# Lillthorin/YoloLite-Official-Repo

Measured on AMD Instinct MI355X. Metric: images/sec, higher is better.
Workload: dtype f32

## Files before the change

include/yololite_hip.h:

```cpp
#ifndef YOLOLITE_HIP_H
#define YOLOLITE_HIP_H

#include <stdint.h>

#ifdef __cplusplus
extern "C" {
#endif

#define YL_ABI_VERSION 7
#define YL_MAX_LEVELS 8

typedef struct yl_ctx yl_ctx;
typedef int32_t yl_status;

enum {
  YL_OK = 0,
  YL_ERR_INVALID = -1,
  YL_ERR_HIP = -2,
  YL_ERR_NOMEM = -3,
  YL_ERR_STATE = -4,
  YL_ERR_UNSUPPORTED = -5,
  YL_ERR_CAPACITY = -6
};

// ... 88 lines not shown

yl_status yl_create(const yl_model_desc* desc, int32_t device_id, yl_ctx** out);
yl_status yl_clone(const yl_ctx* src, yl_ctx** out);
yl_status yl_streams_overlap(int32_t device_id, void* a, void* b, int32_t* overlap);
void yl_destroy(yl_ctx* ctx);
const char* yl_strerror(yl_status s);
const char* yl_last_error(const yl_ctx* ctx);
int32_t yl_abi_version(void);

yl_status yl_forward(yl_ctx* ctx, const float* x_dev, int32_t batch, float* const* level_out_dev,
                     void* stream);
yl_status yl_forward_timed(yl_ctx* ctx, const float* x_dev, int32_t batch, float* const* level_out_dev,
                           void* stream, float* layer_ms);
yl_status yl_last_timing(yl_ctx* ctx, float* infer_ms, float* post_ms);
int64_t yl_activation_bytes(const yl_ctx* ctx);
yl_status yl_read_slot(yl_ctx* ctx, int32_t slot, int32_t batch, float* dst_dev, void* stream);
yl_status yl_set_option(yl_ctx* ctx, const char* name, int32_t value);
yl_status yl_get_option(const yl_ctx* ctx, const char* name, int32_t* value);
int32_t yl_query_fused_block(int32_t c_in, int32_t c_mid, int32_t c_out, int32_t dw_k, int32_t dw_stride, int32_t out_h,
                             int32_t out_w);
int32_t yl_query_ir_form(int32_t c_in, int32_t c_mid, int32_t c_out, int32_t dw_k, int32_t dw_stride, int32_t out_h, int32_t out_w,
                         int32_t batch, int32_t in_h, int32_t in_w, int32_t up_h, int32_t up_w, int32_t act, int32_t dw_act,
                         int32_t act2, int32_t* shape);
int32_t yl_query_dw_prologue(int32_t c_in, int32_t c_out, int32_t dw_k, int32_t dw_stride, int32_t out_h, int32_t out_w);
int32_t yl_query_wino_form(int32_t c_in, int32_t c_out, int32_t out_h, int32_t out_w, int32_t batch, int32_t in_shift,
                           int32_t dev_select, int32_t* mt, int32_t* nt);

typedef struct {
  int64_t offset;
  int32_t h0, w0;
  int32_t nh, nw;
  int32_t top, left;
} yl_pre_image;
yl_status yl_preprocess(yl_ctx* ctx, const uint8_t* packed_u8_dev, const yl_pre_image* imgs_dev, int32_t batch,
                        float* x_dev, void* stream);

yl_status yl_decode(yl_ctx* ctx, const float* const* levels_dev, int32_t batch, int32_t center_mode,
                    int32_t wh_mode, float* box_dev, float* obj_dev, float* cls_dev, void* stream);

yl_status yl_forward_decoded(yl_ctx* ctx, const float* x_dev, int32_t batch, int32_t center_mode, int32_t wh_mode,
                             float* box_dev, float* obj_dev, float* cls_dev, void* stream);

yl_status yl_postprocess(yl_ctx* ctx, const float* const* levels_dev, int32_t batch,
                         const yl_post_cfg* cfg, float* dets_dev, int32_t* counts_dev,
                         int32_t* keep_idx_dev, void* stream);
yl_status yl_predict(yl_ctx* ctx, const float* x_dev, int32_t batch, const yl_post_cfg* cfg,
// ... 424 lines not shown
```

yololite-official-repo_amd/_lib.py:

```python
from __future__ import annotations

import ctypes as C
import os
import sys
import warnings


def _default_hw_queues():
    if "GPU_MAX_HW_QUEUES" in os.environ or os.environ.get("YOLOLITE_NO_ENV_DEFAULTS"):
        return
    os.environ["GPU_MAX_HW_QUEUES"] = "8"
    t = sys.modules.get("torch")
    try:
        late = t is not None and t.cuda.is_initialized()
    except Exception:
        late = False
    if late:
        warnings.warn("yololite_amd: the HIP runtime was initialised before this package was imported, so "
                      "GPU_MAX_HW_QUEUES=8 cannot be applied; export it in the environment (multi-stream overlap "
                      "of the executor degrades by ~25 % next to RCCL streams otherwise)", RuntimeWarning)


_default_hw_queues()

_HERE = os.path.dirname(os.path.abspath(__file__))
LIB_PATH = os.environ.get("YOLOLITE_HIP_LIB") or os.path.join(_HERE, "libyololite_hip.so")

YL_ABI_VERSION = 7
YL_MAX_LEVELS = 8
YL_OK = 0
ACT = {"none": 0, "relu": 1, "relu6": 2, "silu": 3, "gelu": 4, "relu_lab": 5}
OP_STEM, OP_CONV, OP_DW, OP_STEMBLOCK, OP_SE = 0, 1, 2, 3, 4
OP_POOL, OP_COPY, OP_LN, OP_GRN, OP_NHWC4 = 5, 6, 7, 8, 9
POST_MAIN, POST_FALLBACK, POST_EVAL = 0, 1, 2
CENTER = {"v8": 0, "simple": 1}
WH = {"softplus": 0, "v8": 1, "exp": 2}
NMS_TORCHVISION, NMS_GREEDY = 0, 1

DEV_DW_TILE_OFF, DEV_PWS_OFF, DEV_S2C_OFF, DEV_DWC_ALL, DEV_DWT_OFF = 1, 2, 4, 8, 16
DEV_DWT_NOSPLIT = 1 << 10
DEV_WINO_V1 = 1 << 11
DEV_DWL_OFF = 1 << 14
DEV_DWL_ALL = 1 << 15
DEV_DPW_OFF = 1 << 16
DEV_K3W_OFF = 1 << 17
DEV_POISON = 1 << 18
DEV_CHAIN_OFF = 1 << 19
DEV_HEAD_SKIP_OFF = 1 << 20
DEV_PWX_OFF = 1 << 21
DEV_WINO_SHAPE_SHIFT = 12

_fp = C.POINTER(C.c_float)
_ip = C.POINTER(C.c_int32)


class yl_layer(C.Structure):
    _fields_ = [(n, C.c_int32) for n in (
        "op", "in_slot", "out_slot", "res_slot", "up_slot", "head_level", "cin", "cout",
        "k", "stride", "pad_t", "pad_l", "act", "in_shift", "dw_k", "dw_stride", "dw_pad_t", "dw_pad_l", "dw_act")] + [
        ("w", _fp), ("b", _fp), ("dw_w", _fp), ("dw_b", _fp),
        ("c2", C.c_int32), ("act2", C.c_int32), ("c3", C.c_int32), ("act3", C.c_int32),
        ("w2", _fp), ("b2", _fp), ("w3", _fp), ("b3", _fp), ("scale_slot", C.c_int32), ("reserved0", C.c_int32),
        ("lab_scale", C.c_float), ("lab_bias", C.c_float), ("eps", C.c_float), ("out_ch_off", C.c_int32)]


class yl_model_desc(C.Structure):
    _fields_ = [("abi_version", C.c_int32), ("img_size", C.c_int32), ("in_channels", C.c_int32),
                ("num_classes", C.c_int32), ("num_masks", C.c_int32), ("proto_slot", C.c_int32),
                ("num_levels", C.c_int32),
                ("level_size", C.c_int32 * YL_MAX_LEVELS), ("level_anchors", C.c_int32 * YL_MAX_LEVELS),
                ("num_slots", C.c_int32), ("slot_h", _ip), ("slot_w", _ip), ("slot_c", _ip),
                ("num_layers", C.c_int32), ("layers", C.POINTER(yl_layer))]
# ... 189 lines not shown


_vp = C.c_void_p
_vpp = C.POINTER(C.c_void_p)
SYMBOLS = [
    ("yl_create", C.c_int32, [C.POINTER(yl_model_desc), C.c_int32, C.POINTER(_vp)]),
    ("yl_clone", C.c_int32, [_vp, C.POINTER(_vp)]),
    ("yl_streams_overlap", C.c_int32, [C.c_int32, _vp, _vp, C.POINTER(C.c_int32)]),
    ("yl_destroy", None, [_vp]),
    ("yl_strerror", C.c_char_p, [C.c_int32]),
    ("yl_last_error", C.c_char_p, [_vp]),
    ("yl_abi_version", C.c_int32, []),
    ("yl_forward", C.c_int32, [_vp, _vp, C.c_int32, _vpp, _vp]),
    ("yl_forward_timed", C.c_int32, [_vp, _vp, C.c_int32, _vpp, _vp, _fp]),
    ("yl_last_timing", C.c_int32, [_vp, _fp, _fp]),
    ("yl_activation_bytes", C.c_int64, [_vp]),
    ("yl_read_slot", C.c_int32, [_vp, C.c_int32, C.c_int32, _vp, _vp]),
    ("yl_set_option", C.c_int32, [_vp, C.c_char_p, C.c_int32]),
    ("yl_get_option", C.c_int32, [_vp, C.c_char_p, _ip]),
    ("yl_query_fused_block", C.c_int32, [C.c_int32] * 7),
    ("yl_query_dw_prologue", C.c_int32, [C.c_int32] * 6),
    ("yl_query_wino_form", C.c_int32, [C.c_int32] * 7 + [_ip, _ip]),
    ("yl_query_ir_form", C.c_int32, [C.c_int32] * 15 + [_ip]),
    ("yl_forward_decoded", C.c_int32, [_vp, _vp, C.c_int32, C.c_int32, C.c_int32, _vp, _vp, _vp, _vp]),
    ("yl_preprocess", C.c_int32, [_vp, _vp, _vp, C.c_int32, _vp, _vp]),
    ("yl_decode", C.c_int32, [_vp, _vpp, C.c_int32, C.c_int32, C.c_int32, _vp, _vp, _vp, _vp]),
    ("yl_postprocess", C.c_int32, [_vp, _vpp, C.c_int32, C.POINTER(yl_post_cfg), _vp, _vp, _vp, _vp]),
    ("yl_predict", C.c_int32, [_vp, _vp, C.c_int32, C.POINTER(yl_post_cfg), _vp, _vp, _vp, _vp]),
    ("yl_allgather_dets", C.c_int32, [_vp, _vp, _vp, C.c_int64, _vp, _vp]),
    ("yl_masks", C.c_int32, [_vp, _vpp, C.c_int32, _vp, _vp, C.c_int32, C.c_float, _vp, _vp]),
    ("yl_masks_image", C.c_int32, [_vp, _vpp, C.c_int32, _vp, _vp, _vp, C.c_int32, C.c_float, _vp, _vp, _vp, C.c_int32,
                                   C.c_int32, C.c_int32, _vp, _vp]),
    ("yl_nms", C.c_int32, [_vp, _vp, _vp, C.c_int32, C.c_float, C.c_int32, C.c_int32, _vp, _vp, _vp]),
    ("yl_eval_match", C.c_int32, [_vp, _vp, _vp, _vp, C.c_int32, C.c_int32, C.c_double, _vp, _vp, _vp, _vp]),
    ("yl_eval_sweep", C.c_int32, [_vp, _vp, _vp, C.c_int32, _vp, C.c_int32, _vp, _vp, _vp]),
    ("yl_eval_confusion", C.c_int32, [_vp, _vp, _vp, _vp, _vp, _vp, C.c_int32, C.c_int32, C.c_int32, C.c_float,
                                      _vp, _vp, _vp]),
    ("yl_eval_coco_match", C.c_int32, [_vp, _vp, _vp, _vp, _vp, _vp, C.c_int32, C.c_int32, C.c_int32, _vp, C.c_int32,
                                       _vp, C.c_int32, _vp, _vp, _vp]),
    ("yl_eval_coco_accumulate", C.c_int32, [_vp, _vp, _vp, _vp, C.c_int32, _vp, C.c_int32, C.c_int32, C.c_int32, _vp,
                                            C.c_int32, _vp, C.c_int32, _vp, _vp, _vp]),
    ("yl_loss_af", C.c_int32, [_vp, _vpp, C.c_int32, _vp, _vp, _vp, C.c_int32, C.POINTER(yl_loss_cfg), _vp, _vp, _vp, _vp]),
    ("yl_loss_af_train", C.c_int32, [_vp, _vpp, C.c_int32, _vp, _vp, _vp, C.c_int32, C.POINTER(yl_loss_cfg), _vp, _vp, _vp,
                                     _vp, _vp]),
    ("yl_loss_af_backward", C.c_int32, [_vp, _vpp, C.c_int32, _vp, _vp, _vp, C.c_int32, C.POINTER(yl_loss_cfg), _vp, _vp,
                                        _vp, _vpp, _vp]),
# ... 48 lines not shown
                                       _ip]),
    ("yl_stem_plan", C.c_int32, [C.POINTER(yl_stem_cfg), C.c_int32, C.c_int32, C.POINTER(yl_stem_plan_info)]),
    ("yl_stem_create", C.c_int32, [C.c_int32, C.POINTER(yl_stem_cfg), C.POINTER(_vp)]),
    ("yl_stem_destroy", None, [_vp]),
    ("yl_stem_held", C.c_int32, [_vp, C.POINTER(C.c_int64), C.POINTER(C.c_int64), _ip]),
    ("yl_stem_forward", C.c_int32, [_vp, C.POINTER(yl_stem_tensors), _vp, C.c_int32, C.c_int32, C.c_uint32, _vp, _vp, _ip]),
    ("yl_stem_backward", C.c_int32, [_vp, C.POINTER(yl_stem_tensors), C.POINTER(yl_stem_tensors), _vp, _vp, _vp, _ip]),
    ("yl_stem_conv", C.c_int32, [_vp, _vp, _vp] + [C.c_int32] * 8 + [_vp, _ip]),
    ("yl_amp_stage_set", C.c_int32, [_vp, C.c_uint32]),
    ("yl_amp_stem_set", C.c_int32, [_vp, C.c_uint32]),
    ("yl_amp_stage_get", C.c_int32, [_vp, C.POINTER(C.c_uint32), C.POINTER(C.c_uint32)]),
    ("yl_amp_stem_get", C.c_int32, [_vp, C.POINTER(C.c_uint32), C.POINTER(C.c_uint32)]),
    ("yl_amp_stem_conv", C.c_int32, [_vp, _vp, _vp] + [C.c_int32] * 8 + [C.c_uint32, _vp, _ip]),
    ("yl_variant_stage_set", C.c_int32, [_vp, C.c_int32, C.c_int32]),
    ("yl_variant_stage_get", C.c_int32, [_vp, _ip, _ip]),
    ("yl_variant_stage_depthwise", C.c_int32, [_vp, _vp, _vp, C.c_int32, C.c_int32, C.c_int32, C.c_int32, C.c_int32, C.c_int32,
                                               C.c_int32, _vp, _ip]),
    ("yl_augment", C.c_int32, [_vp, _vp, _vp, C.c_int32, C.c_int32, _vp, _vp]),
]
SYMBOLS_DIGITS = [
    ("yl_dneck_conv3x3", C.c_int32, [_vp, C.c_int32, C.c_uint32, _vp, _vp, _vp, C.c_int32, C.c_int32, _vp, _ip]),
]

_lib = None


class YoloLiteHipError(RuntimeError):
    pass


def load():
    global _lib
    if _lib is not None:
        return _lib
    if not os.path.exists(LIB_PATH):
        raise YoloLiteHipError(
            f"{LIB_PATH} not found: build it with `python yololite-official-repo_amd/csrc/build.py` "
            "(or __graft_entry__.build()). There is no CPU fallback.")
    import torch
    try:
        lib = C.CDLL(LIB_PATH, mode=C.RTLD_GLOBAL)
    except OSError as e:
        raise YoloLiteHipError(f"cannot load {LIB_PATH}: {e}") from e
    for name, res, args in SYMBOLS + SYMBOLS_DIGITS:
        fn = getattr(lib, name)
        fn.restype = res
        fn.argtypes = args
    if lib.yl_abi_version() != YL_ABI_VERSION:
        raise YoloLiteHipError("libyololite_hip.so ABI version mismatch")
    _lib = lib
    return lib


def check(status: int, ctx=None, what: str = ""):
    if status == YL_OK:
        return
    lib = load()
    msg = lib.yl_strerror(status).decode()
    detail = lib.yl_last_error(ctx).decode() if ctx else ""
    raise YoloLiteHipError(f"{what or 'yololite_hip'}: {msg} ({status}) {detail}".strip())
```

yololite-official-repo_amd/csrc/yl_api.hip:

```cpp
#include "yl_internal.h"
#include "yl_program.h"

#include <dlfcn.h>
#include <limits.h>
#include <math.h>
#include <stdio.h>
#include <stddef.h>
#include <string.h>

#include <algorithm>
#include <memory>
#include <chrono>
#include <string>
#include <vector>

namespace {

struct DevLayer : YlLayerInfo {
#define YL_X(name) float* name = nullptr;
  YL_LAYER_IMAGES(YL_X)
#undef YL_X
};

struct Slot {
// ... 1227 lines not shown
    unsigned v = 0;
    if (c->head_skip_cnt &&
        (hipSetDevice(c->m->device) != hipSuccess || hipDeviceSynchronize() != hipSuccess ||
         hipMemcpy(&v, c->head_skip_cnt, sizeof(v), hipMemcpyDeviceToHost) != hipSuccess))
      return YL_ERR_HIP;
    *value = (int32_t)(v & 0x7fffffffu);
    return YL_OK;
  }
  return YL_ERR_INVALID;
}

int32_t yl_query_fused_block(int32_t c_in, int32_t c_mid, int32_t c_out, int32_t dw_k, int32_t dw_stride, int32_t out_h,
                             int32_t out_w) {
  if (c_in < 1 || c_mid < 1 || c_out < 1 || out_h < 1 || out_w < 1) return 0;
  if (yl_ir_supported(c_in, c_mid, c_out, dw_k, dw_stride, out_h, out_w)) return 1;
  if (dw_stride == 1 && !(out_h & 3) && !(out_w & 3) && yl_uib_supported(c_in, c_mid, c_out, dw_k)) return 2;
  return 0;
}

int32_t yl_query_ir_form(int32_t c_in, int32_t c_mid, int32_t c_out, int32_t dw_k, int32_t dw_stride, int32_t out_h, int32_t out_w,
                         int32_t batch, int32_t in_h, int32_t in_w, int32_t up_h, int32_t up_w, int32_t act, int32_t dw_act,
                         int32_t act2, int32_t* shape) {
  if (c_in < 1 || c_mid < 1 || c_out < 1 || out_h < 1 || out_w < 1 || batch < 1 || in_h < 1 || in_w < 1 || up_h < 0 || up_w < 0) return 0;
  return yl_ir_form(c_in, c_mid, c_out, dw_k, dw_stride, out_h, out_w, batch, in_h, in_w, up_h, up_w, act, dw_act, act2, shape);
}

int32_t yl_query_dw_prologue(int32_t c_in, int32_t c_out, int32_t dw_k, int32_t dw_stride, int32_t out_h, int32_t out_w) {
  if (c_in < 1 || c_out < 1 || dw_k < 1 || dw_stride < 1 || out_h < 1 || out_w < 1) return 0;
  if (yl_dws_supported(c_in, c_out, dw_k, dw_stride, out_h, out_w)) return 2;
  if ((size_t)(dw_k * dw_k + 1) * c_in * sizeof(float) <= YL_DW_LDS_MAX) return 1;
  return 0;
}

int32_t yl_query_wino_form(int32_t c_in, int32_t c_out, int32_t out_h, int32_t out_w, int32_t batch, int32_t in_shift,
                           int32_t dev_select, int32_t* mt, int32_t* nt) {
  if (mt) *mt = 0;
  if (nt) *nt = 0;
  if (c_in < 16 || c_out < 16 || (c_in & 3) || (c_out & 3)) return 0;
  const unsigned dev = (unsigned)dev_select;
  const YlWinoForm f = yl_wino_form(c_in, c_out, out_h, out_w, batch, in_shift, sizeof(float), (dev & YL_DEV_WINO_V1) != 0, YL_DEV_WINO_SHAPE(dev));
  if (f.form == 2) {
    if (mt) *mt = f.mt;
    if (nt) *nt = f.nt;
  }
  return f.form;
}

// ... 304 lines not shown
```

yololite-official-repo_amd/csrc/yl_convc.hip:

```cpp
#include "yl_lp.h"
#if YL_BF16
#define yl_conv_dwc_kernel YL_LP_NAME(yl_conv_dwc_kernel)
#define yl_launch_conv_dwc YL_LP_NAME(yl_launch_conv_dwc)
#define yl_convc_init YL_LP_NAME(yl_convc_init)
#define yl_conv_pwt_kernel YL_LP_NAME(yl_conv_pwt_kernel)
#define yl_launch_conv_pwt YL_LP_NAME(yl_launch_conv_pwt)
#define yl_launch_conv_pwt_multi YL_LP_NAME(yl_launch_conv_pwt_multi)
#define yl_conv_dwt_kernel YL_LP_NAME(yl_conv_dwt_kernel)
#define yl_launch_conv_dwt YL_LP_NAME(yl_launch_conv_dwt)
#define yl_conv_dwk_kernel YL_LP_NAME(yl_conv_dwk_kernel)
#define yl_conv_dwl_kernel YL_LP_NAME(yl_conv_dwl_kernel)
#define yl_launch_conv_dwk YL_LP_NAME(yl_launch_conv_dwk)
#define yl_conv_dws_kernel YL_LP_NAME(yl_conv_dws_kernel)
#define yl_launch_conv_dws YL_LP_NAME(yl_launch_conv_dws)
#define yl_conv_wino_kernel YL_LP_NAME(yl_conv_wino_kernel)
#define yl_launch_conv_wino YL_LP_NAME(yl_launch_conv_wino)
#define yl_conv_kxk_kernel YL_LP_NAME(yl_conv_kxk_kernel)
#define yl_launch_conv_kxk YL_LP_NAME(yl_launch_conv_kxk)
#define yl_conv_pws_kernel YL_LP_NAME(yl_conv_pws_kernel)
#define yl_launch_conv_pws YL_LP_NAME(yl_launch_conv_pws)
#define yl_ir_kernel YL_LP_NAME(yl_ir_kernel)
#define yl_launch_conv_ir YL_LP_NAME(yl_launch_conv_ir)
#define yl_ir_supported YL_LP_NAME(yl_ir_supported)
#define yl_ir_form YL_LP_NAME(yl_ir_form)
// ... 1324 lines not shown
  const int gy = (p.NTtot + NT - 1) / NT;
  const bool eight = ((long)p.M / 128) * gy >= 2 * 2 * YL_NUM_CU;
  return pws_go(p, st, cand, eight);
}

constexpr __host__ __device__ int yl_ir_pitch(int dk, int ds, int mt, int cbn) { return ((((4 * mt * cbn - 1) * ds + dk) * 16 + 7) / 64) * 64 + 56; }
constexpr __host__ __device__ int yl_ir_slab(int dk, int ds, int mt, int rbn, int cbn) { return ((4 * rbn - 1) * ds + dk) * yl_ir_pitch(dk, ds, mt, cbn); }
struct YlIrLds {
  static constexpr size_t LIMIT = 150 * 1024;
  size_t wpl, dwl, b2l, bytes;
  constexpr __host__ __device__ YlIrLds(int dk, int ds, int mt, int rbn, int cbn, int nt, int KB)
      : wpl((size_t)2 * yl_ir_slab(dk, ds, mt, rbn, cbn)), dwl(wpl + (size_t)2 * nt * 256), b2l(dwl + (size_t)KB * (dk * dk + 1) * 16),
        bytes((b2l + (size_t)KB * 16) * 4) {}
};

template <bool CLAMP>
__device__ __forceinline__ f32x4 yl_ir_act(f32x4 v, int act, float lo, float hi) {
  if constexpr (CLAMP) return yl_clamp4(v, lo, hi);
  else return yl_actc(v, act, lo, hi);
}
constexpr int yl_ir_waves(int kbi, int nt, int dk, int ds, int mt, bool clamp) {
  return (dk == 3 && ds * mt <= 2 && kbi <= 3 && (nt <= 3 || (clamp && ds * mt == 1))) ? 3 : 2;
}
template <int KBI , int NT, int DK, int DS, int MT, int RBN , int CBN , bool CLAMP>
__global__ __launch_bounds__(RBN * CBN * 64, yl_ir_waves(KBI, NT, DK, DS, MT, CLAMP)) void yl_ir_kernel(YlConvP p) {
  constexpr int NWV = RBN * CBN, NTH = NWV * 64;
  constexpr int TH = 4 * RBN, TW = 4 * MT * CBN;
  constexpr int HH = (TH - 1) * DS + DK, HW = (TW - 1) * DS + DK, HN = HH * HW;
  constexpr int HMT = (HN + 15) / 16, HMW = (HMT + NWV - 1) / NWV;
  constexpr int PITCHF = yl_ir_pitch(DK, DS, MT, CBN), SLAB = yl_ir_slab(DK, DS, MT, RBN, CBN);
  extern __shared__ __attribute__((aligned(16))) float yl_clds[];
  const int tid = threadIdx.x, lane = tid & 63;
  const int wave = __builtin_amdgcn_readfirstlane(tid >> 6);
  const int kq = lane >> 4, pl = lane & 15;
  const int Cmid = p.Cin, KB = p.KB, NTtot = p.NTtot, C1 = p.C1, H = p.H, W = p.W, OH = p.OH, OW = p.OW, N = p.N;
  const YlIrLds L(DK, DS, MT, RBN, CBN, NT, KB);
  float* slab = yl_clds;
  f32x4* wpl = reinterpret_cast<f32x4*>(yl_clds + L.wpl);
  float* dwl = yl_clds + L.dwl;
  float* b2l = yl_clds + L.b2l;
  const f32x4* wg = reinterpret_cast<const f32x4*>(p.wp);
  const f32x4* w2g = reinterpret_cast<const f32x4*>(p.w2p);
  const yl_act_t* const xin = p.x;
  const yl_act_t* const up = p.up;
  {
    constexpr int T1 = DK * DK + 1;
    for (int i = tid; i < KB * T1 * 16; i += NTH) {
      const int kb = i / (T1 * 16), r = i - kb * (T1 * 16), t = r >> 4, ch = kb * 16 + (r & 15);
// ... 105 lines not shown
      for (int nt = 0; nt < NT; ++nt) {
        acc[mt][nt] = (f32x4){0.f, 0.f, 0.f, 0.f};
        const int n = nt * 16 + 4 * kq;
        if (pre_add && n < N) acc[mt][nt] = yl_ld4(p.res + px[mt].lin * N + n);
      }
    f32x4 we[KBI], wn[KBI];
#pragma unroll
    for (int kbi = 0; kbi < KBI; ++kbi) {
      if constexpr (CLAMP) wn[kbi] = __builtin_bit_cast(f32x4, __builtin_amdgcn_raw_buffer_load_b128(wrs, lane16, kbi * KB * 1024, 0));
      else wn[kbi] = w2g[((size_t)kbi * KB + 0) * 64 + lane];
    }
    f32x4 un[HMW];
    auto load_up = [&](int kb, int j) {
      if constexpr (CLAMP) {
        return bld4(urs, (kb + 1 < KB || kb * 16 + 4 * kq < Cmid) ? uo[j] : OOR, kb * 16 * ESZ);
      } else {
        return yl_ld4((h_in[j] && kb * 16 + 4 * kq < Cmid) ? up + uoff[j] + kb * 16 : p.zeros);
      }
    };
    if (up) {
#pragma unroll
      for (int j = 0; j < HMW; ++j) un[j] = load_up(0, j);
    }
    for (int kb = 0; kb < KB; ++kb, ++gs) {
      const int buf = (int)(gs & 1u);
#pragma unroll
      for (int kbi = 0; kbi < KBI; ++kbi) we[kbi] = wn[kbi];
      if (kb + 1 < KB) {
#pragma unroll
        for (int kbi = 0; kbi < KBI; ++kbi) {
          if constexpr (CLAMP) wn[kbi] = __builtin_bit_cast(f32x4, __builtin_amdgcn_raw_buffer_load_b128(wrs, lane16, (kbi * KB + kb + 1) * 1024, 0));
          else wn[kbi] = w2g[((size_t)kbi * KB + kb + 1) * 64 + lane];
        }
      }
      const f32x4 eb = yl_ld4(b2l + kb * 16 + 4 * kq);
      float* sb = slab + buf * SLAB;
#pragma unroll
      for (int j = 0; j < HMW; ++j) {
        f32x4 e[1][1] = {{{0.f, 0.f, 0.f, 0.f}}};
        if (up) e[0][0] = un[j];
#pragma unroll
        for (int kbi = 0; kbi < KBI; ++kbi) {
          const f32x4 wq1[1] = {we[kbi]};
          const f32x4 xq1[1] = {xh[j][kbi]};
          yl_mma_step<1, 1>(wq1, xq1, e);
        }
// ... 15 lines not shown
#pragma unroll
          for (int mt = 0; mt < MT; ++mt) {
            const f32x4 v = *reinterpret_cast<const f32x4*>(sb + rbase + dy * PITCHF + (dx + 4 * mt * DS) * 16);
            xq[mt].x = fmaf(v.x, w.x, xq[mt].x); xq[mt].y = fmaf(v.y, w.y, xq[mt].y);
            xq[mt].z = fmaf(v.z, w.z, xq[mt].z); xq[mt].w = fmaf(v.w, w.w, xq[mt].w);
          }
        }
      };
#pragma unroll 1
      for (int dy = 0; dy < DK; ++dy) tap_row(dy);
#pragma unroll
      for (int mt = 0; mt < MT; ++mt) xq[mt] = yl_ir_act<CLAMP>(xq[mt], dw_act, dlo, dhi);
      f32x4 wq[NT];
      const f32x4* wrow = wpl + (size_t)buf * NT * 64 + lane;
#pragma unroll
      for (int nt = 0; nt < NT; ++nt) wq[nt] = wrow[nt * 64];
      yl_mma_step<NT, MT>(wq, xq, acc);
    }
    if (!pre_add && (p.res || (!CLAMP && YL_SMOOTH(p.act)))) yl_epi_generic<NT, MT>(p, acc, px, 0, kq);
    else yl_epi_fast<NT, MT>(p, acc, px, 0, kq, lo, hi, true);
  }
}

template <int KBI, int NT, int DK, int DS, int MT, int RBN, int CBN, bool CLAMP>
static hipError_t ir_go(const YlConvP& p, hipStream_t st, bool second) {
  if (CLAMP && !second) return hipErrorNotSupported;
  const size_t lds = YlIrLds(DK, DS, MT, RBN, CBN, NT, p.KB).bytes;
  const long ntiles = (long)p.B * (p.OH / (4 * RBN)) * (p.OW / (4 * MT * CBN));
  int gx = yl_resident_blocks((const void*)yl_ir_kernel<KBI, NT, DK, DS, MT, RBN, CBN, CLAMP>, RBN * CBN * 64, lds, 8);
  if (gx > ntiles) gx = (int)ntiles;
  if (gx >= 8) gx &= ~7;
  hipLaunchKernelGGL((yl_ir_kernel<KBI, NT, DK, DS, MT, RBN, CBN, CLAMP>), dim3(gx), dim3(RBN * CBN * 64), lds, st, p);
  return hipGetLastError();
}

#define YL_IR_SHAPES(X)                                                                                              \
  X(1, 2, 3, 2, 1, 2, 2) X(2, 2, 3, 1, 2, 2, 2) X(2, 3, 5, 2, 1, 2, 2) X(3, 3, 5, 1, 2, 2, 2) X(3, 6, 3, 2, 1, 2, 2)    \
  X(3, 3, 3, 1, 1, 2, 2) X(2, 6, 3, 1, 2, 2, 2) X(3, 6, 3, 1, 1, 2, 2)
#define YL_IR_BUCKET_LO(B) ((B) == 2 ? 0 : (B) == 3 ? 2 : (B) == 4 ? 3 : 4)

bool yl_ir_supported(int c1, int cmid, int n, int dk, int ds, int oh, int ow) {
  const int kbi = (c1 + 15) / 16, nt = (n + 15) / 16;
#define YL_IR_CHECK(A, B, C, D, E, R, S)                                                                             \
  if (kbi == A && nt <= B && nt > YL_IR_BUCKET_LO(B) && dk == C && ds == D && (oh % (4 * R)) == 0 &&                    \
      (ow % (4 * E * S)) == 0 && YlIrLds(C, D, E, R, S, B, (cmid + 15) / 16).bytes <= YlIrLds::LIMIT) return true;
  YL_IR_SHAPES(YL_IR_CHECK)
#undef YL_IR_CHECK
  return false;
}

int yl_ir_form(int c1, int cmid, int n, int dk, int ds, int oh, int ow, int batch, int h, int w, int uh, int uw, int act,
               int dw_act, int act2, int* shape) {
  const int kbi = (c1 + 15) / 16, nt = (n + 15) / 16, KB = (cmid + 15) / 16;
  const size_t lim = ((size_t)1 << 31) - 4096, e = sizeof(yl_act_t);
  const bool second = !YL_SMOOTH(act) && !YL_SMOOTH(dw_act) && !YL_SMOOTH(act2) && batch > 0 && h > 0 && w > 0 && uh >= 0 && uw >= 0 &&
                      (size_t)batch * h * w * c1 * e < lim && (size_t)batch * uh * uw * cmid * e < lim &&
                      (size_t)kbi * KB * 1024 < lim && (size_t)KB * nt * 1024 < lim;
#define YL_IR_FORM(A, B, C, D, E, R, S)                                                                              \
  if (kbi == A && nt <= B && nt > YL_IR_BUCKET_LO(B) && dk == C && ds == D && (oh % (4 * R)) == 0 &&                    \
      (ow % (4 * E * S)) == 0 && YlIrLds(C, D, E, R, S, B, KB).bytes <= YlIrLds::LIMIT) {                                \
    const int sh[7] = {A, B, C, D, E, R, S};                                                                         \
    for (int i = 0; shape && i < 7; ++i) shape[i] = sh[i];                                                           \
    return second ? 2 : 1;                                                                                           \
  }
  YL_IR_SHAPES(YL_IR_FORM)
#undef YL_IR_FORM
  return 0;
}

hipError_t yl_launch_conv_ir(const YlConvP& p, hipStream_t st) {
  if (p.C1 <= 0 || p.k != 1 || p.dw_k == 0 || (p.N & 3)) return hipErrorNotSupported;
  const int kbi = (p.C1 + 15) / 16, nt = p.NTtot;
  const bool second = yl_ir_form(p.C1, p.Cin, p.N, p.dw_k, p.dw_stride, p.OH, p.OW, p.B, p.H, p.W, p.up ? p.UH : 0, p.up ? p.UW : 0,
                                 p.act, p.dw_act, p.act2, nullptr) == 2;
#define YL_IR_RUN(A, B, C, D, E, R, S)                                                                               \
  if (kbi == A && nt <= B && nt > YL_IR_BUCKET_LO(B) && p.dw_k == C && p.dw_stride == D && (p.OH % (4 * R)) == 0 &&     \
      (p.OW % (4 * E * S)) == 0 && YlIrLds(C, D, E, R, S, B, p.KB).bytes <= YlIrLds::LIMIT) {                               \
    const hipError_t e2 = ir_go<A, B, C, D, E, R, S, true>(p, st, second);                                           \
    return e2 != hipErrorNotSupported ? e2 : ir_go<A, B, C, D, E, R, S, false>(p, st, second);                        \
  }
  YL_IR_SHAPES(YL_IR_RUN)
#undef YL_IR_RUN
  return hipErrorNotSupported;
}

struct YlDwkLds {
  static constexpr size_t LIMIT = 96 * 1024;
  static constexpr __host__ __device__ int steps(int NT, int GW) { return GW == 1 ? 3 : (GW * NT <= 16 ? 2 : 1); }
  size_t dwl, bytes;
  constexpr __host__ __device__ YlDwkLds(int NT, int GW, int Cin)
      : dwl((size_t)2 * steps(NT, GW) * GW * NT * 256), bytes((dwl + yl_taps_floats(3, Cin)) * 4) {}
};

template <int NT, int GW, int NW>
__global__ __launch_bounds__(NW * 64, GW == 1 ? 3 : 2) void yl_conv_dwk_kernel(YlConvP p) {
  constexpr int S = YlDwkLds::steps(NT, GW);
  constexpr int PCS = S * GW * NT;
// ... 1073 lines not shown
  const int gx = yl_band_grid(yl_resident_blocks((const void*)wino2_kernel_of(MT, NT, 0), 512, lds, 8), (long)p.ntiles * G);
  hipLaunchKernelGGL(wino2_kernel_of(MT, NT, p.in_shift), dim3(gx), dim3(512), lds, st, p);
  return hipGetLastError();
}

hipError_t yl_launch_conv_wino(const YlConvP& p, hipStream_t st) {
  if (!p.wino || p.k != 3 || p.stride != 1 || p.dw_k > 0 || p.up || p.dec_boxes || p.C1 > 0 || p.w3p || p.scale) return hipErrorNotSupported;
  const YlWinoForm f = yl_wino_form(p.Cin, p.N, p.OH, p.OW, p.B,
                                    p.in_shift, sizeof(yl_act_t), (p.dev & YL_DEV_WINO_V1) != 0, YL_DEV_WINO_SHAPE(p.dev));
  if (f.form == 0) return hipErrorNotSupported;
  return f.form == 2 ? wino2_go(p, st, f.mt, f.nt) : wino_go(p, st);
}

namespace {

#define YL_DWC_SHAPES(NTW) \
  {{yl_conv_dwc_kernel<3, 1, NTW>, yl_conv_dwc_kernel<3, 2, NTW>}, {yl_conv_dwc_kernel<5, 1, NTW>, yl_conv_dwc_kernel<5, 2, NTW>}}
const YlMultiKernel dwc_kernels[5][2][2] = {YL_DWC_SHAPES(1), YL_DWC_SHAPES(2), YL_DWC_SHAPES(3), YL_DWC_SHAPES(4), YL_DWC_SHAPES(5)};

int kbmax_of(int ntw) { return ntw == 1 ? 18 : ntw == 2 ? 9 : ntw == 3 ? 6 : 4; }

}

hipError_t yl_convc_init() {
  hipError_t e = hipSuccess;
  const auto cap = [&e](const auto& kernels, size_t bytes) { if (e == hipSuccess) e = yl_set_lds_cap(kernels, bytes); };
#define YL_KXK_CAP(A, B, C) cap(yl_conv_kxk_kernel<A, B, C>, YlKxkLds::LIMIT);
  YL_KXK_SHAPES(YL_KXK_CAP)
#define YL_IR_CAP(A, B, C, D, E, R, S) cap(yl_ir_kernel<A, B, C, D, E, R, S, false>, YlIrLds::LIMIT); cap(yl_ir_kernel<A, B, C, D, E, R, S, true>, YlIrLds::LIMIT);
  YL_IR_SHAPES(YL_IR_CAP)
  cap(pws_kernels, YlPwsLds::LIMIT);
  cap(pws_dec_kernels, YlPwsLds::LIMIT);
  cap(dwt_kernels, YlDwtLds::LIMIT);
  cap(dwt_splitk_kernels, YlDwtLds::LIMIT);
  cap(wino_kernels, YlWinoLds::LIMIT);
#define YL_WINO2_CAP(A, B) cap(yl_conv_wino2_kernel<A, B, 1>, YlWino2Lds(A).bytes); cap(yl_conv_wino2_kernel<A, B, 0>, YlWino2Lds(A).bytes);
  YL_WINO2_SHAPES(YL_WINO2_CAP)
#define YL_DWK_CAP(A, B, C) cap(yl_conv_dwk_kernel<A, B, C>, YlDwkLds::LIMIT);
  YL_DWK_SHAPES(YL_DWK_CAP)
#define YL_DWL_CAP(A) cap(yl_conv_dwl_kernel<A>, YlDwlLds::LIMIT);
  YL_DWL_SHAPES(YL_DWL_CAP)
#define YL_DWS_CAP(A, G, K, S_) cap(yl_conv_dws_kernel<A, G, K, S_, 4>, YlDwsLds::LIMIT);
  YL_DWS_SHAPES(YL_DWS_CAP)
#if !YL_BF16
#define YL_DWX_CAP(A, B) cap(yl_conv_dwx_kernel<A, B>, YlDwtLds::LIMIT);
  YL_DWX_SHAPES(YL_DWX_CAP)
#define YL_PWX_CAP(A, B, C, D) cap(yl_conv_pwx_kernel<A, B, C, D>, YlPwxLds::LIMIT);
  YL_PWX_SHAPES(YL_PWX_CAP)
#undef YL_PWX_CAP
#endif
  cap(dwc_kernels, YlDwcLds::LIMIT);
  return e;
// ... 37 lines not shown
```

yololite-official-repo_amd/csrc/yl_internal.h:

```cpp
#pragma once
#include <hip/hip_runtime.h>
#include <stdint.h>
#include <map>
#include <mutex>
#include <type_traits>
#include <utility>
#include "../../include/yololite_hip.h"
#include "yl_lp.h"
#include "yl_shapes.h"

#define YL_LDS_KEYS_MAX 16384

struct YlLevels {
  const float* ptr[YL_MAX_LEVELS];
  int S[YL_MAX_LEVELS];
  int A[YL_MAX_LEVELS];
  int off[YL_MAX_LEVELS + 1];
  float stride[YL_MAX_LEVELS];
  int L, N, E, C;
  float hi;
};

struct YlDecodeP {
  int mode;
// ... 115 lines not shown
  int ldo;
  int out_f32;
};

#define YL_DEV_DW_TILE_OFF (1u << 0)
#define YL_DEV_PWS_OFF (1u << 1)
#define YL_DEV_S2C_OFF (1u << 2)
#define YL_DEV_DWC_ALL (1u << 3)
#define YL_DEV_DWT_OFF (1u << 4)
#define YL_DEV_DWK(d) (((d) >> 5) & 3u)
#define YL_DEV_KXK_NW(d) (((d) >> 7) & 3u)
#define YL_DEV_KXK_MT2 (1u << 9)
#define YL_DEV_DWT_NOSPLIT (1u << 10)
#define YL_DEV_WINO_V1 (1u << 11)
#define YL_DEV_WINO_SHAPE(d) (((d) >> 12) & 3u)
#define YL_DEV_DWL_OFF (1u << 14)
#define YL_DEV_DWL_ALL (1u << 15)
#define YL_DEV_DPW_OFF (1u << 16)
#define YL_DEV_K3W_OFF (1u << 17)
#define YL_DEV_POISON (1u << 18)
#define YL_DEV_CHAIN_OFF (1u << 19)
#define YL_DEV_HEAD_SKIP_OFF (1u << 20)
#define YL_DEV_PWX_OFF (1u << 21)
#define YL_DEV_MASK 0x3ffffffu
static_assert(YL_DEV_MASK <= 0x7fffffffu, "dev_select is stored in an int (and an int field of the graph key)");
static_assert(((YL_DEV_DW_TILE_OFF | YL_DEV_PWS_OFF | YL_DEV_S2C_OFF | YL_DEV_DWC_ALL | YL_DEV_DWT_OFF | (3u << 5) | (3u << 7) |
                YL_DEV_KXK_MT2 | YL_DEV_DWT_NOSPLIT | YL_DEV_WINO_V1 | (3u << 12) | YL_DEV_DWL_OFF | YL_DEV_DWL_ALL | YL_DEV_DPW_OFF |
                YL_DEV_K3W_OFF | YL_DEV_POISON | YL_DEV_CHAIN_OFF | YL_DEV_HEAD_SKIP_OFF | YL_DEV_PWX_OFF) & ~YL_DEV_MASK) == 0, "a YL_DEV_* bit lies outside the dev_select mask");

struct YlSeP {
  const float* x;
  float* partial;
  const float* w1;
  const float* b1;
  const float* w2;
  const float* b2;
  float* gate;
  int B, HW, C, RD, P, act;
};
hipError_t yl_launch_se(const YlSeP& p, bool pooled, hipStream_t st);
int yl_se_parts(int HW, int C);
int yl_dw_pool_wpi(int k, int stride, int cin, int n, int oh, int ow);

struct YlOpP {
  const float* x;
  float* out;
  const float* w;
  const float* b;
  float* partial;
  int B, H, W, C, OH, OW;
  int k, stride, pad_t, pad_l;
// ... 123 lines not shown
```

yololite-official-repo_amd/csrc/yl_shapes.h:

```cpp
#pragma once

#define YL_SMOOTH(a) ((a) >= YL_ACT_SILU)
#define YL_ACT_POSTPASS(a) ((a) >= YL_ACT_GELU)

#include <stddef.h>

#define YL_NUM_CU 256

bool yl_stemblock_supported(int c1, int c2, int c3);
bool yl_uib_supported(int c1, int cmid, int n, int dk);
bool yl_ir_supported(int c1, int cmid, int n, int dk, int ds, int oh, int ow);
int yl_ir_form(int c1, int cmid, int n, int dk, int ds, int oh, int ow, int batch, int h, int w, int uh, int uw, int act,
               int dw_act, int act2, int* shape);
bool yl_dws_supported(int cin, int n, int dk, int ds, int oh, int ow);

#define YL_WINO2_SHAPES(X) X(4, 3) X(4, 4) X(2, 3) X(2, 4) X(2, 7)

struct YlWinoForm {
  int form;
  int mt, nt;
};

inline YlWinoForm yl_wino_form(int cin, int n, int oh, int ow, int batch, int in_shift, size_t elem, bool v1, unsigned shape) {
  if (cin < 1 || n < 1 || oh < 1 || ow < 1 || batch < 1 || (n & 3) || in_shift < 0 || in_shift > 1 ||
      ((size_t)batch * (oh >> in_shift) * (ow >> in_shift) * cin + (size_t)(ow + 1) * cin) * elem >= ((size_t)1 << 31))
    return {0, 0, 0};
  const int KB = (cin + 15) / 16, NTtot = (n + 15) / 16;
  const bool small = (size_t)batch * (oh >> in_shift) * (ow >> in_shift) * cin * elem < ((size_t)1 << 31) &&
                     (size_t)((NTtot + 1) / 2) * KB * 32768 < ((size_t)1 << 31);
  if (!v1 && KB >= 2 && NTtot >= 3 && small) {
    const int TW = (ow + 1) >> 1, TH = (oh + 1) >> 1;
    const int MX = (TW + 3) >> 2, MY = (TH + 3) >> 2;
    const long MTOT = (long)batch * MX * MY;
    if ((long)TW * TH * 100 >= (long)MX * MY * 16 * 65) {
      const int pad3 = (NTtot + 2) / 3 * 3, pad4 = (NTtot + 3) / 4 * 4;
      int nt = pad3 <= pad4 ? 3 : 4;
// ... 10 lines not shown
```

Before: 51750.

## Pipeline inverted-residual kernel: overlap next expansion MFMA with depthwise taps

Adds a pipelined schedule to the fused inverted-residual kernel for specific shapes (KBI=3, 3x3 depthwise, MT=1). Expansion MFMAs for the next channel block are interleaved with the depthwise tap FMAs of the current block, with the results stored into a double-buffered LDS slab, and sched_group_barrier hints steer the interleaving. The aim is to hide the serial dependency between the expansion and depthwise stages. It adds register pressure and complexity, and a DEV_IR_SERIAL flag plus a query API can disable it or report it.

After: 51940 (median of 6 runs). About the same (+0.4%).

```diff
diff --git a/include/yololite_hip.h b/include/yololite_hip.h
--- a/include/yololite_hip.h
+++ b/include/yololite_hip.h
@@ -134,6 +134,9 @@
 int32_t yl_query_ir_form(int32_t c_in, int32_t c_mid, int32_t c_out, int32_t dw_k, int32_t dw_stride, int32_t out_h, int32_t out_w,
                          int32_t batch, int32_t in_h, int32_t in_w, int32_t up_h, int32_t up_w, int32_t act, int32_t dw_act,
                          int32_t act2, int32_t* shape);
+int32_t yl_query_ir_schedule(int32_t c_in, int32_t c_mid, int32_t c_out, int32_t dw_k, int32_t dw_stride, int32_t out_h, int32_t out_w,
+                             int32_t batch, int32_t in_h, int32_t in_w, int32_t up_h, int32_t up_w, int32_t act, int32_t dw_act,
+                             int32_t act2, int32_t dev_select);
 int32_t yl_query_dw_prologue(int32_t c_in, int32_t c_out, int32_t dw_k, int32_t dw_stride, int32_t out_h, int32_t out_w);
 int32_t yl_query_wino_form(int32_t c_in, int32_t c_out, int32_t out_h, int32_t out_w, int32_t batch, int32_t in_shift,
                            int32_t dev_select, int32_t* mt, int32_t* nt);
diff --git a/yololite-official-repo_amd/_lib.py b/yololite-official-repo_amd/_lib.py
--- a/yololite-official-repo_amd/_lib.py
+++ b/yololite-official-repo_amd/_lib.py
@@ -24,7 +24,8 @@
 _default_hw_queues()
 
 _HERE = os.path.dirname(os.path.abspath(__file__))
-LIB_PATH = os.environ.get("YOLOLITE_HIP_LIB") or os.path.join(_HERE, "libyololite_hip.so")
+_DEFAULT_LIB_PATH = os.path.join(_HERE, "libyololite_hip.so")
+LIB_PATH = os.environ.get("YOLOLITE_HIP_LIB") or _DEFAULT_LIB_PATH
 
 YL_ABI_VERSION = 7
 YL_MAX_LEVELS = 8
@@ -48,6 +49,7 @@
 DEV_CHAIN_OFF = 1 << 19
 DEV_HEAD_SKIP_OFF = 1 << 20
 DEV_PWX_OFF = 1 << 21
+DEV_IR_SERIAL = 1 << 22
 DEV_WINO_SHAPE_SHIFT = 12
 
 _fp = C.POINTER(C.c_float)
@@ -283,6 +285,7 @@
     ("yl_query_dw_prologue", C.c_int32, [C.c_int32] * 6),
     ("yl_query_wino_form", C.c_int32, [C.c_int32] * 7 + [_ip, _ip]),
     ("yl_query_ir_form", C.c_int32, [C.c_int32] * 15 + [_ip]),
+    ("yl_query_ir_schedule", C.c_int32, [C.c_int32] * 16),
     ("yl_forward_decoded", C.c_int32, [_vp, _vp, C.c_int32, C.c_int32, C.c_int32, _vp, _vp, _vp, _vp]),
     ("yl_preprocess", C.c_int32, [_vp, _vp, _vp, C.c_int32, _vp, _vp]),
     ("yl_decode", C.c_int32, [_vp, _vpp, C.c_int32, C.c_int32, C.c_int32, _vp, _vp, _vp, _vp]),
@@ -377,6 +380,8 @@
     ("yl_dneck_conv3x3", C.c_int32, [_vp, C.c_int32, C.c_uint32, _vp, _vp, _vp, C.c_int32, C.c_int32, _vp, _ip]),
 ]
 
+QUERIES_NOT_IN_PARENT = {"yl_query_ir_schedule"}
+
 _lib = None
 
 
@@ -398,6 +403,8 @@
     except OSError as e:
         raise YoloLiteHipError(f"cannot load {LIB_PATH}: {e}") from e
     for name, res, args in SYMBOLS + SYMBOLS_DIGITS:
+        if name in QUERIES_NOT_IN_PARENT and LIB_PATH != _DEFAULT_LIB_PATH and not hasattr(lib, name):
+            continue
         fn = getattr(lib, name)
         fn.restype = res
         fn.argtypes = args
diff --git a/yololite-official-repo_amd/csrc/yl_api.hip b/yololite-official-repo_amd/csrc/yl_api.hip
--- a/yololite-official-repo_amd/csrc/yl_api.hip
+++ b/yololite-official-repo_amd/csrc/yl_api.hip
@@ -1273,7 +1273,17 @@
                          int32_t batch, int32_t in_h, int32_t in_w, int32_t up_h, int32_t up_w, int32_t act, int32_t dw_act,
                          int32_t act2, int32_t* shape) {
   if (c_in < 1 || c_mid < 1 || c_out < 1 || out_h < 1 || out_w < 1 || batch < 1 || in_h < 1 || in_w < 1 || up_h < 0 || up_w < 0) return 0;
-  return yl_ir_form(c_in, c_mid, c_out, dw_k, dw_stride, out_h, out_w, batch, in_h, in_w, up_h, up_w, act, dw_act, act2, shape);
+  return yl_ir_form(c_in, c_mid, c_out, dw_k, dw_stride, out_h, out_w, batch, in_h, in_w, up_h, up_w, act, dw_act, act2, shape, 0u, nullptr);
+}
+
+int32_t yl_query_ir_schedule(int32_t c_in, int32_t c_mid, int32_t c_out, int32_t dw_k, int32_t dw_stride, int32_t out_h, int32_t out_w,
+                             int32_t batch, int32_t in_h, int32_t in_w, int32_t up_h, int32_t up_w, int32_t act, int32_t dw_act,
+                             int32_t act2, int32_t dev_select) {
+  if (c_in < 1 || c_mid < 1 || c_out < 1 || out_h < 1 || out_w < 1 || batch < 1 || in_h < 1 || in_w < 1 || up_h < 0 || up_w < 0) return 0;
+  int sched = 0;
+  const int form = yl_ir_form(c_in, c_mid, c_out, dw_k, dw_stride, out_h, out_w, batch, in_h, in_w, up_h, up_w, act, dw_act, act2, nullptr,
+                              (unsigned)dev_select, &sched);
+  return form == 0 ? 0 : 1 + sched;
 }
 
 int32_t yl_query_dw_prologue(int32_t c_in, int32_t c_out, int32_t dw_k, int32_t dw_stride, int32_t out_h, int32_t out_w) {
diff --git a/yololite-official-repo_amd/csrc/yl_convc.hip b/yololite-official-repo_amd/csrc/yl_convc.hip
--- a/yololite-official-repo_amd/csrc/yl_convc.hip
+++ b/yololite-official-repo_amd/csrc/yl_convc.hip
@@ -1370,8 +1370,16 @@
 constexpr int yl_ir_waves(int kbi, int nt, int dk, int ds, int mt, bool clamp) {
   return (dk == 3 && ds * mt <= 2 && kbi <= 3 && (nt <= 3 || (clamp && ds * mt == 1))) ? 3 : 2;
 }
-template <int KBI , int NT, int DK, int DS, int MT, int RBN , int CBN , bool CLAMP>
+constexpr bool yl_ir_pipe(int kbi, int nt, int dk, int ds, int mt) {
+#if YL_BF16
+  return false;
+#else
+  return kbi == 3 && dk == 3 && mt == 1 && ((nt == 3 && ds == 1) || (nt == 6 && ds == 2));
+#endif
+}
+template <int KBI , int NT, int DK, int DS, int MT, int RBN , int CBN , bool CLAMP, bool PIPE = false>
 __global__ __launch_bounds__(RBN * CBN * 64, yl_ir_waves(KBI, NT, DK, DS, MT, CLAMP)) void yl_ir_kernel(YlConvP p) {
+  static_assert(CLAMP || !PIPE, "the pipelined schedule exists for the second form only");
   constexpr int NWV = RBN * CBN, NTH = NWV * 64;
   constexpr int TH = 4 * RBN, TW = 4 * MT * CBN;
   constexpr int HH = (TH - 1) * DS + DK, HW = (TW - 1) * DS + DK, HN = HH * HW;
@@ -1523,6 +1531,120 @@
 #pragma unroll
       for (int j = 0; j < HMW; ++j) un[j] = load_up(0, j);
     }
+    if constexpr (PIPE) {
+      if (!up) {
+#pragma unroll
+        for (int j = 0; j < HMW; ++j) un[j] = (f32x4){0.f, 0.f, 0.f, 0.f};
+      }
+      f32x4 e[HMW][1];
+      auto e_mma = [&](int kbi) {
+        const f32x4 wq1[1] = {wn[kbi]};
+        f32x4 xq1[HMW];
+#pragma unroll
+        for (int j = 0; j < HMW; ++j) xq1[j] = xh[j][kbi];
+        yl_mma_step<1, HMW>(wq1, xq1, e);
+      };
+      auto e_next = [&](int kb) {
+        if (kb < KB) {
+#pragma unroll
+          for (int kbi = 0; kbi < KBI; ++kbi)
+            wn[kbi] = __builtin_bit_cast(f32x4, __builtin_amdgcn_raw_buffer_load_b128(wrs, lane16, (kbi * KB + kb) * 1024, 0));
+          if (up) {
+#pragma unroll
+            for (int j = 0; j < HMW; ++j) un[j] = load_up(kb, j);
+          }
+        }
+      };
+      auto e_store = [&](int kb, int buf) {
+        const f32x4 eb = yl_ld4(b2l + kb * 16 + 4 * kq);
+        float* sb = slab + buf * SLAB;
+#pragma unroll
+        for (int j = 0; j < HMW; ++j) {
+          const f32x4 v = yl_sel4(h_in[j], yl_ir_act<CLAMP>(e[j][0] + eb, act2, elo, ehi));
+          if (h_ok[j]) *reinterpret_cast<f32x4*>(sb + h_lo[j]) = v;
+        }
+      };
+#pragma unroll
+      for (int j = 0; j < HMW; ++j) e[j][0] = un[j];
+#pragma unroll
+      for (int kbi = 0; kbi < KBI; ++kbi) e_mma(kbi);
+      e_next(1);
+      e_store(0, (int)(gs & 1u));
+      for (int kb = 0; kb < KB; ++kb, ++gs) {
+        const int buf = (int)(gs & 1u);
+        const float* sb = slab + buf * SLAB;
+        __builtin_amdgcn_s_waitcnt(0x0F70);
+        __syncthreads();
+        const float* tapw = dwl + kb * ((DK * DK + 1) * 16) + 4 * kq;
+        f32x4 xq[MT];
+#pragma unroll
+        for (int mt = 0; mt < MT; ++mt) xq[mt] = yl_ld4(tapw + DK * DK * 16);
+        auto tap_fma = [&](const f32x4 (&tw)[DK], const f32x4 (&tv)[DK][MT]) {
+#pragma unroll
+          for (int dx = 0; dx < DK; ++dx)
+#pragma unroll
+            for (int mt = 0; mt < MT; ++mt) {
+              xq[mt].x = fmaf(tv[dx][mt].x, tw[dx].x, xq[mt].x); xq[mt].y = fmaf(tv[dx][mt].y, tw[dx].y, xq[mt].y);
+              xq[mt].z = fmaf(tv[dx][mt].z, tw[dx].z, xq[mt].z); xq[mt].w = fmaf(tv[dx][mt].w, tw[dx].w, xq[mt].w);
+            }
+        };
+        auto tap_read = [&](int dy, f32x4 (&tw)[DK], f32x4 (&tv)[DK][MT]) {
+#pragma unroll
+          for (int dx = 0; dx < DK; ++dx) {
+            tw[dx] = yl_ld4(tapw + (dy * DK + dx) * 16);
+#pragma unroll
+            for (int mt = 0; mt < MT; ++mt) tv[dx][mt] = *reinterpret_cast<const f32x4*>(sb + rbase + dy * PITCHF + (dx + 4 * mt * DS) * 16);
+          }
+        };
+        if (kb + 1 < KB) {
+          constexpr int M = YL_MFMA_PER_BLOCK * HMW, T = M >= 2 ? 2 : 1, F = DK * MT * 4;
+#pragma unroll
+          for (int j = 0; j < HMW; ++j) e[j][0] = un[j];
+#pragma unroll
+          for (int dy = 0; dy < DK; ++dy) {
+            __builtin_amdgcn_sched_barrier(0);
+            f32x4 tw[DK], tv[DK][MT];
+            tap_read(dy, tw, tv);
+            if (dy < KBI) e_mma(dy);
+            tap_fma(tw, tv);
+#pragma unroll
+            for (int mt = 0; mt < MT; ++mt) asm volatile("" : "+v"(xq[mt]));
+            __builtin_amdgcn_sched_group_barrier(0x100, DK * (1 + MT), 0);
+            if (dy < KBI) {
+              if (M > T) __builtin_amdgcn_sched_group_barrier(0x008, M - T, 0);
+#pragma unroll
+              for (int t = 0; t < T; ++t) {
+                __builtin_amdgcn_sched_group_barrier(0x008, 1, 0);
+                __builtin_amdgcn_sched_group_barrier(0x002, (F + T - 1) / T, 0);
+              }
+            } else {
+              __builtin_amdgcn_sched_group_barrier(0x002, F, 0);
+            }
+          }
+#pragma unroll
+          for (int kbi = DK; kbi < KBI; ++kbi) e_mma(kbi);
+          __builtin_amdgcn_sched_barrier(0);
+          load_proj(kb + 1, buf ^ 1);
+          e_next(kb + 2);
+          e_store(kb + 1, buf ^ 1);
+        } else {
+          if (tile + tstride < tend) load_proj(0, buf ^ 1);
+#pragma unroll 1
+          for (int dy = 0; dy < DK; ++dy) {
+            f32x4 tw[DK], tv[DK][MT];
+            tap_read(dy, tw, tv);
+            tap_fma(tw, tv);
+          }
+        }
+#pragma unroll
+        for (int mt = 0; mt < MT; ++mt) xq[mt] = yl_ir_act<CLAMP>(xq[mt], dw_act, dlo, dhi);
+        f32x4 wq[NT];
+        const f32x4* wrow = wpl + (size_t)buf * NT * 64 + lane;
+#pragma unroll
+        for (int nt = 0; nt < NT; ++nt) wq[nt] = wrow[nt * 64];
+        yl_mma_step<NT, MT>(wq, xq, acc);
+      }
+    } else
     for (int kb = 0; kb < KB; ++kb, ++gs) {
       const int buf = (int)(gs & 1u);
 #pragma unroll
@@ -1584,15 +1706,18 @@
   }
 }
 
-template <int KBI, int NT, int DK, int DS, int MT, int RBN, int CBN, bool CLAMP>
+template <int KBI, int NT, int DK, int DS, int MT, int RBN, int CBN, bool CLAMP, bool PIPE = false>
 static hipError_t ir_go(const YlConvP& p, hipStream_t st, bool second) {
   if (CLAMP && !second) return hipErrorNotSupported;
+  if constexpr (CLAMP && !PIPE && yl_ir_pipe(KBI, NT, DK, DS, MT)) {
+    if (!(p.dev & YL_DEV_IR_SERIAL)) return ir_go<KBI, NT, DK, DS, MT, RBN, CBN, true, true>(p, st, second);
+  }
   const size_t lds = YlIrLds(DK, DS, MT, RBN, CBN, NT, p.KB).bytes;
   const long ntiles = (long)p.B * (p.OH / (4 * RBN)) * (p.OW / (4 * MT * CBN));
-  int gx = yl_resident_blocks((const void*)yl_ir_kernel<KBI, NT, DK, DS, MT, RBN, CBN, CLAMP>, RBN * CBN * 64, lds, 8);
+  int gx = yl_resident_blocks((const void*)yl_ir_kernel<KBI, NT, DK, DS, MT, RBN, CBN, CLAMP, PIPE>, RBN * CBN * 64, lds, 8);
   if (gx > ntiles) gx = (int)ntiles;
   if (gx >= 8) gx &= ~7;
-  hipLaunchKernelGGL((yl_ir_kernel<KBI, NT, DK, DS, MT, RBN, CBN, CLAMP>), dim3(gx), dim3(RBN * CBN * 64), lds, st, p);
+  hipLaunchKernelGGL((yl_ir_kernel<KBI, NT, DK, DS, MT, RBN, CBN, CLAMP, PIPE>), dim3(gx), dim3(RBN * CBN * 64), lds, st, p);
   return hipGetLastError();
 }
 
@@ -1612,7 +1737,7 @@
 }
 
 int yl_ir_form(int c1, int cmid, int n, int dk, int ds, int oh, int ow, int batch, int h, int w, int uh, int uw, int act,
-               int dw_act, int act2, int* shape) {
+               int dw_act, int act2, int* shape, unsigned dev, int* sched) {
   const int kbi = (c1 + 15) / 16, nt = (n + 15) / 16, KB = (cmid + 15) / 16;
   const size_t lim = ((size_t)1 << 31) - 4096, e = sizeof(yl_act_t);
   const bool second = !YL_SMOOTH(act) && !YL_SMOOTH(dw_act) && !YL_SMOOTH(act2) && batch > 0 && h > 0 && w > 0 && uh >= 0 && uw >= 0 &&
@@ -1623,6 +1748,7 @@
       (ow % (4 * E * S)) == 0 && YlIrLds(C, D, E, R, S, B, KB).bytes <= YlIrLds::LIMIT) {                                \
     const int sh[7] = {A, B, C, D, E, R, S};                                                                         \
     for (int i = 0; shape && i < 7; ++i) shape[i] = sh[i];                                                           \
+    if (sched) *sched = (second && yl_ir_pipe(A, B, C, D, E) && !(dev & YL_DEV_IR_SERIAL)) ? 1 : 0;                  \
     return second ? 2 : 1;                                                                                           \
   }
   YL_IR_SHAPES(YL_IR_FORM)
@@ -1634,7 +1760,7 @@
   if (p.C1 <= 0 || p.k != 1 || p.dw_k == 0 || (p.N & 3)) return hipErrorNotSupported;
   const int kbi = (p.C1 + 15) / 16, nt = p.NTtot;
   const bool second = yl_ir_form(p.C1, p.Cin, p.N, p.dw_k, p.dw_stride, p.OH, p.OW, p.B, p.H, p.W, p.up ? p.UH : 0, p.up ? p.UW : 0,
-                                 p.act, p.dw_act, p.act2, nullptr) == 2;
+                                 p.act, p.dw_act, p.act2, nullptr, p.dev, nullptr) == 2;
 #define YL_IR_RUN(A, B, C, D, E, R, S)                                                                               \
   if (kbi == A && nt <= B && nt > YL_IR_BUCKET_LO(B) && p.dw_k == C && p.dw_stride == D && (p.OH % (4 * R)) == 0 &&     \
       (p.OW % (4 * E * S)) == 0 && YlIrLds(C, D, E, R, S, B, p.KB).bytes <= YlIrLds::LIMIT) {                               \
@@ -2754,12 +2880,18 @@
 
 }
 
+template <int KBI, int NT, int DK, int DS, int MT, int RBN, int CBN, class Cap>
+static void ir_pipe_cap(const Cap& cap) {
+  if constexpr (yl_ir_pipe(KBI, NT, DK, DS, MT)) cap(yl_ir_kernel<KBI, NT, DK, DS, MT, RBN, CBN, true, true>, YlIrLds::LIMIT);
+}
+
 hipError_t yl_convc_init() {
   hipError_t e = hipSuccess;
   const auto cap = [&e](const auto& kernels, size_t bytes) { if (e == hipSuccess) e = yl_set_lds_cap(kernels, bytes); };
 #define YL_KXK_CAP(A, B, C) cap(yl_conv_kxk_kernel<A, B, C>, YlKxkLds::LIMIT);
   YL_KXK_SHAPES(YL_KXK_CAP)
-#define YL_IR_CAP(A, B, C, D, E, R, S) cap(yl_ir_kernel<A, B, C, D, E, R, S, false>, YlIrLds::LIMIT); cap(yl_ir_kernel<A, B, C, D, E, R, S, true>, YlIrLds::LIMIT);
+#define YL_IR_CAP(A, B, C, D, E, R, S) cap(yl_ir_kernel<A, B, C, D, E, R, S, false>, YlIrLds::LIMIT); cap(yl_ir_kernel<A, B, C, D, E, R, S, true>, YlIrLds::LIMIT); \
+  ir_pipe_cap<A, B, C, D, E, R, S>(cap);
   YL_IR_SHAPES(YL_IR_CAP)
   cap(pws_kernels, YlPwsLds::LIMIT);
   cap(pws_dec_kernels, YlPwsLds::LIMIT);
diff --git a/yololite-official-repo_amd/csrc/yl_internal.h b/yololite-official-repo_amd/csrc/yl_internal.h
--- a/yololite-official-repo_amd/csrc/yl_internal.h
+++ b/yololite-official-repo_amd/csrc/yl_internal.h
@@ -161,11 +161,12 @@
 #define YL_DEV_CHAIN_OFF (1u << 19)
 #define YL_DEV_HEAD_SKIP_OFF (1u << 20)
 #define YL_DEV_PWX_OFF (1u << 21)
+#define YL_DEV_IR_SERIAL (1u << 22)
 #define YL_DEV_MASK 0x3ffffffu
 static_assert(YL_DEV_MASK <= 0x7fffffffu, "dev_select is stored in an int (and an int field of the graph key)");
 static_assert(((YL_DEV_DW_TILE_OFF | YL_DEV_PWS_OFF | YL_DEV_S2C_OFF | YL_DEV_DWC_ALL | YL_DEV_DWT_OFF | (3u << 5) | (3u << 7) |
                 YL_DEV_KXK_MT2 | YL_DEV_DWT_NOSPLIT | YL_DEV_WINO_V1 | (3u << 12) | YL_DEV_DWL_OFF | YL_DEV_DWL_ALL | YL_DEV_DPW_OFF |
-                YL_DEV_K3W_OFF | YL_DEV_POISON | YL_DEV_CHAIN_OFF | YL_DEV_HEAD_SKIP_OFF | YL_DEV_PWX_OFF) & ~YL_DEV_MASK) == 0, "a YL_DEV_* bit lies outside the dev_select mask");
+                YL_DEV_K3W_OFF | YL_DEV_POISON | YL_DEV_CHAIN_OFF | YL_DEV_HEAD_SKIP_OFF | YL_DEV_PWX_OFF | YL_DEV_IR_SERIAL) & ~YL_DEV_MASK) == 0, "a YL_DEV_* bit lies outside the dev_select mask");
 
 struct YlSeP {
   const float* x;
diff --git a/yololite-official-repo_amd/csrc/yl_shapes.h b/yololite-official-repo_amd/csrc/yl_shapes.h
--- a/yololite-official-repo_amd/csrc/yl_shapes.h
+++ b/yololite-official-repo_amd/csrc/yl_shapes.h
@@ -11,7 +11,7 @@
 bool yl_uib_supported(int c1, int cmid, int n, int dk);
 bool yl_ir_supported(int c1, int cmid, int n, int dk, int ds, int oh, int ow);
 int yl_ir_form(int c1, int cmid, int n, int dk, int ds, int oh, int ow, int batch, int h, int w, int uh, int uw, int act,
-               int dw_act, int act2, int* shape);
+               int dw_act, int act2, int* shape, unsigned dev, int* sched);
 bool yl_dws_supported(int cin, int n, int dk, int ds, int oh, int ow);
 
 #define YL_WINO2_SHAPES(X) X(4, 3) X(4, 4) X(2, 3) X(2, 4) X(2, 7)
```
